# 0xC0000054/pdn-jpegxl

Hardware: AMD Instinct MI355X
Metric: megapixels/sec decode (4K lossy VarDCT) (higher is better)
Workload: dtype f32

## Files before the change

pdn_jpegxl_amd/csrc/decoder.cc:

```cpp
#include <hip/hip_runtime.h>
#include <algorithm>
#include <atomic>
#include <cmath>
#include <cstdarg>
#include <cstdio>
#include <cstdlib>
#include <cstring>
#include <memory>
#include <mutex>
#include <string>
#include <thread>
#include <vector>
#include "../../include/jxlfiletypeio.h"
#include "host_parse.h"
#include "icc.h"
#include "kernels.h"

namespace jxlhip {

struct HipError : std::runtime_error {
  explicit HipError(const std::string& m) : std::runtime_error(m) {}
};
#define HIP_OK(expr)                                                                                      \
  do {                                                                                                    \
// ... 77 lines not shown
  hipStream_t own_stream = nullptr;
  float* d_basis_all = nullptr;
  float* d_basis_small = nullptr;
  float* d_basis_mfma = nullptr;
  float* d_llf_scale = nullptr;
  uint16_t* d_natural[kNumOrders] = {};
  U32x2* d_scan[kNumQuantTables] = {};
  float* d_dq[kNumQuantTables] = {};
  uint32_t dq_n[kNumQuantTables] = {};
  struct Tap { std::vector<uint8_t> qcoef[3], xyb_idct[3], xyb_filtered[3], noise_rnd[3], noise[3]; };
  struct Slot {
    uint8_t* d_ws = nullptr; size_t ws_cap = 0;
    uint8_t* d_blob = nullptr; size_t blob_cap = 0;
    uint8_t* h_blob = nullptr; size_t h_blob_cap = 0;
    uint32_t* h_status = nullptr; size_t h_status_cap = 0;
    int n = 0;
    std::vector<ParsedFrame> frames;
    int nfiles = 0;
    std::vector<int> file_of;
    std::vector<ParsedFrame> files;
    std::vector<DevImage> imgs;
    std::vector<int> parse_status;
    std::vector<std::string> parse_msg;
    std::vector<size_t> status_off;
    DevImage* d_imgs = nullptr;
    bool pending = false;
    hipEvent_t lf_done = nullptr, hf_done = nullptr, done = nullptr, uploaded = nullptr;
    std::vector<Tap> taps;
    std::vector<std::string> stage_names;
    std::vector<int> stage_chain;
    std::vector<hipEvent_t> events;
    std::vector<float> stage_ms;
  };
  static constexpr int kSlots = 3;
  static constexpr int kPixelChunk = 32;
  Slot slots[kSlots];
  int cur = 0, last = 0;
  Slot* active = &slots[0];
  hipStream_t stream_lf = nullptr;
  hipStream_t stream_hf = nullptr;
  hipStream_t last_stream = nullptr;
  std::vector<std::string> total_names;
  std::vector<double> total_ms;
  int total_batches = 0;
  std::string sticky_error;
  int sticky_status = 0;
  uint8_t* li_dev = nullptr; uint8_t* li_host = nullptr; size_t li_cap = 0;
  void EnsureLoadImageBuffers(size_t bytes);
  int lane_stride_override = 0;
  int hf_stride_override = 0;
  bool debug_taps = false;
  int band_first_row = 0, band_rows = 0;
  bool no_stream_pairs = false;
  bool no_direct = false, mod_lanes64 = false;
  bool overlap = true;

  explicit JxlHipDecoder(int dev);
  ~JxlHipDecoder();
  void EnsureWs(size_t bytes);
  void EnsureBlob(size_t bytes);
  void Mark(const char* name, hipStream_t s, int chain);
  void WaitSlot(Slot& S);
  Slot& Last() { return slots[last]; }
  void Decode(int32_t n_, const uint8_t* const* host_data, const size_t* sizes, const uint8_t* const* dev_data,
              uint8_t* const* dev_out, hipStream_t stream, bool sync, DecoderStatus* statuses, ErrorInfo* err);
  DecoderStatus Finish(DecoderStatus* statuses, ErrorInfo* err);
  void CopyPlaneTap(int stage);
  void PrepassSingle(ParsedFrame& f, const uint8_t* dev_file);
};

JxlHipDecoder::JxlHipDecoder(int dev) {
  if (dev < 0) HIP_OK(hipGetDevice(&dev));
  device = dev;
  HIP_OK(hipSetDevice(device));
  int entropy_cus = 0, pixel_cus = 0;
  if (const char* e = Knob("JXLHIP_ENTROPY_CUS")) entropy_cus = std::min(256, std::max(0, atoi(e)));
  if (const char* e = Knob("JXLHIP_PIXEL_CUS")) pixel_cus = std::min(256, std::max(0, atoi(e)));
  auto masked_stream = [](hipStream_t* s, int first, int count) {
    uint32_t mask[8] = {0, 0, 0, 0, 0, 0, 0, 0};
    for (int i = first; i < first + count; i++) mask[i >> 5] |= 1u << (i & 31);
    HIP_OK(hipExtStreamCreateWithCUMask(s, 8, mask));
  };
  if (pixel_cus) masked_stream(&own_stream, 256 - pixel_cus, pixel_cus);
  else HIP_OK(hipStreamCreateWithFlags(&own_stream, hipStreamNonBlocking));
  int prio_least = 0, prio_greatest = 0;
  (void)hipDeviceGetStreamPriorityRange(&prio_least, &prio_greatest);
  const int prio = Knob("JXLHIP_NO_PRIORITY") ? prio_least : prio_greatest;
  if (entropy_cus) {
    masked_stream(&stream_lf, 0, entropy_cus);
    masked_stream(&stream_hf, 0, entropy_cus);
  } else {
    HIP_OK(hipStreamCreateWithPriority(&stream_lf, hipStreamNonBlocking, prio));
    HIP_OK(hipStreamCreateWithPriority(&stream_hf, hipStreamNonBlocking, prio));
  }
  for (auto& S : slots) {
    HIP_OK(hipEventCreateWithFlags(&S.lf_done, hipEventDisableTiming));
    HIP_OK(hipEventCreateWithFlags(&S.hf_done, hipEventDisableTiming));
    HIP_OK(hipEventCreateWithFlags(&S.done, hipEventDisableTiming));
    HIP_OK(hipEventCreateWithFlags(&S.uploaded, hipEventDisableTiming));
  }
  if (const char* e = Knob("JXLHIP_NO_OVERLAP")) overlap = atoi(e) == 0;
  const StaticTables& st = GetStaticTables();
  std::vector<float> all;
  for (int i = 0; i < 6; i++) all.insert(all.end(), st.basis[i].begin(), st.basis[i].end());
  HIP_OK(hipMalloc(&d_basis_all, all.size() * 4));
  HIP_OK(hipMemcpy(d_basis_all, all.data(), all.size() * 4, hipMemcpyHostToDevice));
// ... 1026 lines not shown
      }
    }
  }
  if (!patch_tiles.empty()) {
    PatchFrame* pfr = (PatchFrame*)(h_blob + off_patch_frames);
    for (size_t k = 0; k < patch_image.size(); k++) {
      const ParsedFrame& f = frames[patch_image[k]];
      PatchFrame& p = pfr[k];
      memset(&p, 0, sizeof(p));
      p.px = (float*)imgs[patch_image[k]].out;
      p.w = (int32_t)f.xsize; p.h = (int32_t)f.ysize;
      p.has_alpha = f.alpha_index >= 0 ? 1 : 0;
      p.nch = f.ncolor + p.has_alpha;
      p.premul = (p.has_alpha && f.ec[f.alpha_index].alpha_associated) ? 1 : 0;
    }
    for (size_t k = 0; k < patch_refs.size(); k++) {
      const HostPatchRef& s = patch_src[k];
      const ParsedFrame& a = frames[s.atlas];
      const size_t nch = a.ncolor + (a.alpha_index >= 0 ? 1 : 0);
      patch_refs[k].px = (const float*)imgs[s.atlas].out + ((size_t)s.y0 * a.xsize + s.x0) * nch;
      patch_refs[k].stride = (int32_t)a.xsize;
    }
    memcpy(h_blob + off_patch_refs, patch_refs.data(), sizeof(PatchRef) * patch_refs.size());
    memcpy(h_blob + off_patch_pos, patch_pos.data(), sizeof(PatchPos) * patch_pos.size());
    memcpy(h_blob + off_patch_tiles, patch_tiles.data(), sizeof(PatchTile) * patch_tiles.size());
    memcpy(h_blob + off_patch_list, patch_list.data(), sizeof(int32_t) * patch_list.size());
  }
  memcpy(h_blob + off_imgs, imgs.data(), sizeof(DevImage) * imgs.size());
  d_imgs = (DevImage*)(d_blob + off_imgs);
  stage_names.clear();
  S.stage_chain.clear();
  Mark("start", s_lf, 0);
  static const int skip_stages = Knob("JXLHIP_SKIP_STAGES") ? atoi(Knob("JXLHIP_SKIP_STAGES")) : 0;
  if (!(skip_stages & 1)) HIP_OK(hipMemsetAsync(d_ws, 0, zero_bytes, s_lf));
  HIP_OK(hipMemcpyAsync(d_blob, h_blob, blob.off, hipMemcpyHostToDevice, s_lf));
  Mark("upload+clear", s_lf, 0);
  const bool pix_on_hf = Knob("JXLHIP_PIX_ON_HF") && s_hf != stream;
  const bool early_noise = any_noise && !debug_taps && s_lf != stream && !pix_on_hf;
  if (early_noise) {
    HIP_OK(hipEventRecord(S.uploaded, s_lf));
    HIP_OK(hipStreamWaitEvent(stream, S.uploaded, 0));
    Mark("noise_start", stream, 3);
    LaunchNoise(d_imgs, std::min(pixel_chunk, n), max_groups, max_w, max_h, stream);
    Mark("noise", stream, 3);
  }
  const int direct_lf = global_direct && lf_per_wave == 1, direct_alpha = global_direct && per_alpha_wg == 1;
  bool lean_mod = true;
  for (int i = 0; i < n; i++)
    if (parse_status[i] == DecoderStatus_Ok && frames[i].encoding == 0 &&
        (!frames[i].tree_row_static || frames[i].tree_uses_wp || frames[i].mcode.use_prefix || frames[i].mcode.lz77)) lean_mod = false;
  if (!(skip_stages & 1)) {
  LaunchLfAns(d_imgs, (const SectionTask*)(d_blob + off_lf_ans_tasks), nlf_ans_t, lf_per_wave, lds_lf <= kLdsMax ? lds_lf : 0, direct_lf, lean_mod, s_lf);
  Mark("lf_ans", s_lf, 0);
  LaunchLfFinish(d_imgs, (const SectionTask*)(d_blob + off_lf_tasks), nlf_t, s_lf);
  LaunchHfBlockList(d_imgs, n, max_groups, s_lf);
  LaunchLfPixelStages(d_imgs, n, max_cells, s_lf);
  }
  Mark("lf_finish+pixels", s_lf, 0);
  if (s_lf != s_hf) {
    HIP_OK(hipEventRecord(S.lf_done, s_lf));
    HIP_OK(hipStreamWaitEvent(s_hf, S.lf_done, 0));
  }
#ifdef JXLHIP_EXPERIMENTS
  if (const char* e = Knob("JXLHIP_INTERFERE")) {
    int kind = 0, wgs = 1, lds_kb = 64; float ms = 100.f;
    if (sscanf(e, "%d,%d,%d,%f", &kind, &wgs, &lds_kb, &ms) >= 1 && kind >= 1 && kind <= 6 && wgs >= 1 && wgs <= 16 && lds_kb >= 1 && lds_kb <= 160 && ms > 0 && ms < 2000) {
      static hipStream_t xs = nullptr;
      static float* xbuf = nullptr;
      const size_t xbytes = (size_t)512 << 20;
      if (!xs) { HIP_OK(hipStreamCreateWithFlags(&xs, hipStreamNonBlocking)); HIP_OK(hipMalloc(&xbuf, xbytes)); }
      if (s_lf != s_hf) HIP_OK(hipStreamWaitEvent(xs, S.lf_done, 0));
      LaunchInterference(kind, wgs, lds_kb, ms, xbuf, xbytes, xs);
    }
  }
#endif
  Mark("hf_start", s_hf, 1);
  if (!(skip_stages & 2))
  LaunchHfDecode(d_imgs, (const SectionTask*)(d_blob + off_pass_tasks), npass_t, hf_waves * 64, lane_stride, hf_ring, lds_hf <= kLdsMax ? lds_hf : 0, lds_hf_lanes, s_hf);
  Mark("hf_decode", s_hf, 1);
  if (any_alpha && !(skip_stages & 4))
    LaunchAlphaAns(d_imgs, (const SectionTask*)(d_blob + off_alpha_tasks), nalpha_t, alpha_stride, lds_alpha <= kLdsMax ? lds_alpha : 0, direct_alpha, lean_mod, s_hf);
  Mark("alpha_ans", s_hf, 1);
  if (debug_taps) {
    taps.assign(n, Tap());
    LaunchExpandCoefficients(d_imgs, n, true, max_tiles, stream);
    HIP_OK(hipStreamSynchronize(stream));
    CopyPlaneTap(0);
  }
  const bool finish_on_hf = s_hf == stream || debug_taps || !Knob("JXLHIP_ALPHA_FINISH_ON_PIX");
  if (finish_on_hf) {
    if (any_alpha && !(skip_stages & 4)) LaunchAlphaFinish(d_imgs, n, max_groups, s_hf);
    Mark("alpha_finish", s_hf, 1);
  }
  if (s_hf != stream) {
    HIP_OK(hipEventRecord(S.hf_done, s_hf));
    HIP_OK(hipStreamWaitEvent(stream, S.hf_done, 0));
  }
  Mark("main_start", stream, 2);
  if (!finish_on_hf) {
    if (any_alpha && !(skip_stages & 4)) LaunchAlphaFinish(d_imgs, n, max_groups, stream);
    Mark("alpha_finish", stream, 2);
  }
  hipStream_t s_pix = pix_on_hf ? s_hf : stream;
  for (int c0 = 0; c0 < n; c0 += pixel_chunk) {
    const int cnt = std::min(pixel_chunk, n - c0);
    if (!(skip_stages & 8))
    LaunchReconTiles(d_imgs + c0, cnt, max_tiles, d_basis_all, d_basis_small, d_llf_scale, d_basis_mfma, s_pix);
// ... 257 lines not shown
    info->has_alpha = f.alpha_index >= 0;
    info->num_channels = f.ncolor + (f.black_index >= 0 ? 1 : 0) + info->has_alpha;
    info->bytes_per_sample = (int32_t)OutBytesPerSample(f);
    info->reserved = f.exp_bits ? 1 : 0;
    info->xsize_blocks = f.w8; info->ysize_blocks = f.h8;
    info->num_groups = f.ng; info->num_lf_groups = f.nlf;
    info->epf_iters = f.epf_iters; info->gaborish = f.gab;
    info->codestream_bytes = f.cs_size;
    return DecoderStatus_Ok;
  } catch (const ParseError& e) {
    SetErr(err, "%s", e.what());
    return e.status;
  } catch (const std::exception& e) {
    SetErr(err, "%s", e.what());
    return DecoderStatus_DecodeError;
  }
}

DecoderStatus jxlhip_decode_batch(JxlHipDecoder* dec, int32_t n, const uint8_t* const* host_data, const size_t* sizes,
                                  const uint8_t* const* dev_data, uint8_t* const* dev_out, void* stream, int32_t synchronize,
                                  DecoderStatus* statuses, ErrorInfo* err) {
  if (!dec || !host_data || !sizes || !dev_out || n <= 0) return DecoderStatus_NullParameter;
  try {
    dec->Decode(n, host_data, sizes, dev_data, dev_out, (hipStream_t)stream, synchronize != 0, statuses, err);
    if (statuses) for (int i = 0; i < n; i++) if (statuses[i] != DecoderStatus_Ok) return statuses[i];
    return DecoderStatus_Ok;
  } catch (const std::bad_alloc&) {
    return DecoderStatus_OutOfMemory;
  } catch (const std::exception& e) {
    SetErr(err, "%s", e.what());
    return DecoderStatus_DecodeError;
  }
}

DecoderStatus jxlhip_finish(JxlHipDecoder* dec, DecoderStatus* statuses, ErrorInfo* err) {
  if (!dec) return DecoderStatus_NullParameter;
  try {
    return dec->Finish(statuses, err);
  } catch (const std::exception& e) {
    SetErr(err, "%s", e.what());
    return DecoderStatus_DecodeError;
  }
}

int32_t jxlhip_set_option(JxlHipDecoder* dec, const char* name, int32_t value) {
  if (!dec || !name) return 0;
  if (!strcmp(name, "debug_taps")) { dec->debug_taps = value != 0; return 1; }
  if (!strcmp(name, "query_pixel_chunk")) return JxlHipDecoder::kPixelChunk;
  if (!strcmp(name, "lane_stride")) { if (value != 0 && !PowerOfTwoUpTo64(value)) return 0; dec->lane_stride_override = value; return 1; }
  if (!strcmp(name, "band_first_row")) { if (value < 0) return 0; dec->band_first_row = value; return 1; }
  if (!strcmp(name, "band_rows")) { if (value < 0) return 0; dec->band_rows = value; return 1; }
  if (!strcmp(name, "no_direct")) { dec->no_direct = value != 0; return 1; }
  if (!strcmp(name, "no_stream_pairs")) { dec->no_stream_pairs = value != 0; return 1; }
  if (!strcmp(name, "mod_lanes64")) { dec->mod_lanes64 = value != 0; return 1; }
  if (!strcmp(name, "overlap")) { dec->overlap = value != 0; return 1; }
  return 0;
}

size_t jxlhip_read_plane(JxlHipDecoder* dec, int32_t index, const char* name, int32_t channel, void* dst, size_t capacity) {
  if (!dec || !name) return 0;
  JxlHipDecoder::Slot& S = dec->Last();
  if (index < 0 || index >= S.n || S.pending) return 0;
  if (S.parse_status[index] != DecoderStatus_Ok) return 0;
  const DevImage& d = S.imgs[index];
  std::string nm(name);
  const size_t cells = (size_t)d.w8 * d.h8, pix = (size_t)d.wp * d.hp;
  const void* src = nullptr;
  size_t bytes = 0;
  bool host = false;
  const int c = std::min(2, std::max(0, channel));
  if (nm == "lf") { src = d.lf_final[c]; bytes = cells * 4; }
  else if (nm == "lf_quant") { src = d.lfq[c]; bytes = cells * 4; }
  else if (nm == "cellinfo") { src = d.cellinfo; bytes = cells * 4; }
  else if (nm == "raw_quant") { src = d.rawq; bytes = cells * 2; }
  else if (nm == "sharpness") { src = d.sharp; bytes = cells; }
  else if (nm == "ytox") { src = d.ytox; bytes = (size_t)d.wt * d.ht; }
  else if (nm == "ytob") { src = d.ytob; bytes = (size_t)d.wt * d.ht; }
  else if (nm == "alpha") { src = d.alpha; bytes = (size_t)d.w * d.h; }
  else if (nm == "inv_sigma") { src = d.inv_sigma; bytes = cells * 4; }
  else if (dec->debug_taps && (size_t)index < S.taps.size()) {
    host = true;
    if (nm == "qcoef") { src = S.taps[index].qcoef[c].data(); bytes = S.taps[index].qcoef[c].size(); }
    else if (nm == "xyb_idct") { src = S.taps[index].xyb_idct[c].data(); bytes = S.taps[index].xyb_idct[c].size(); }
    else if (nm == "xyb_filtered") { src = S.taps[index].xyb_filtered[c].data(); bytes = S.taps[index].xyb_filtered[c].size(); }
    else if (nm == "noise_rnd") { src = S.taps[index].noise_rnd[c].data(); bytes = S.taps[index].noise_rnd[c].size(); }
    else if (nm == "noise") { src = S.taps[index].noise[c].data(); bytes = S.taps[index].noise[c].size(); }
  }
  (void)pix;
  if (!src || !bytes) return 0;
  if (dst && capacity) {
    size_t nb = std::min(bytes, capacity);
    if (host) memcpy(dst, src, nb);
    else if (hipMemcpy(dst, src, nb, hipMemcpyDeviceToHost) != hipSuccess) return 0;
  }
  return bytes;
}

int32_t jxlhip_stage_times(JxlHipDecoder* dec, const char** names, float* ms, int32_t capacity) {
  if (!dec) return 0;
  JxlHipDecoder::Slot& S = dec->Last();
  int32_t k = 0;
  for (size_t i = 1; i < S.stage_names.size() && i < S.stage_ms.size() && k < capacity; i++) {
    if (S.stage_ms[i] < 0.f) continue;
    if (names) names[k] = S.stage_names[i].c_str();
    if (ms) ms[k] = S.stage_ms[i];
    k++;
// ... 209 lines not shown
```

pdn_jpegxl_amd/csrc/entropy_kernels.hip:

```cpp
#include <hip/hip_runtime.h>
#include <cstdlib>
#include "dev_types.h"
#include "dev_util.h"
#include "kernels.h"

namespace jxlhip {

namespace {

__device__ const uint8_t d_order_bucket[kNumStrategies] = {0, 1, 1, 1, 2, 3, 4, 4, 5, 5, 6, 6, 1, 1, 1, 1, 1, 1, 7, 8, 8, 9, 10, 10, 11, 12, 12};
__device__ const uint8_t d_log2cx[kNumStrategies] = {0, 0, 0, 0, 1, 2, 0, 1, 0, 2, 1, 2, 0, 0, 0, 0, 0, 0, 3, 2, 3, 4, 3, 4, 5, 4, 5};
__device__ const uint8_t d_log2cy[kNumStrategies] = {0, 0, 0, 0, 1, 2, 1, 0, 2, 0, 2, 1, 0, 0, 0, 0, 0, 0, 3, 3, 2, 4, 4, 3, 5, 5, 4};
__device__ const uint8_t d_nnz_ctx[64] = {0,   0,   31,  62,  62,  93,  93,  93,  93,  123, 123, 123, 123, 152, 152, 152, 152, 152, 152, 152, 152, 180,
                                          180, 180, 180, 180, 180, 180, 180, 180, 180, 180, 180, 206, 206, 206, 206, 206, 206, 206, 206, 206, 206, 206,
                                          206, 206, 206, 206, 206, 206, 206, 206, 206, 206, 206, 206, 206, 206, 206, 206, 206, 206, 206, 206};

__device__ __forceinline__ int CeilLog2D(uint32_t x) { return x <= 1 ? 0 : 32 - __clz(x - 1); }
__device__ __forceinline__ int32_t UnpackSigned(uint32_t u) { return (int32_t)(u >> 1) ^ -(int32_t)(u & 1); }
#ifndef JXLHIP_PRIO_SERIAL
#define JXLHIP_PRIO_SERIAL 0
#endif
#if JXLHIP_PRIO_SERIAL
#define JXL_SERIAL_PRIO() __builtin_amdgcn_s_setprio(JXLHIP_PRIO_SERIAL)
#else
// ... 1013 lines not shown
      if (b.Read(4) != 3) { err |= kErrUnsupportedHeader; break; }
      b.SetLz(lzw, 20, max(max((uint32_t)tw, count), (uint32_t)bw));
      b.lz_copy = 0; b.lz_done = 0;
      state = InitAnsState(b, mt.tab);
    }
    int chan, sid, w, h, stride;
    int32_t* out;
    ChanDesc* cd = desc + max(i, 0);
    if (i < 0) {
      chan = 0; sid = 0; w = im.w; h = im.h; stride = im.w; out = im.alpha32; cd = im.alpha_desc;
    } else if (i < 3) {
      const int c = i == 0 ? 1 : (i == 1 ? 0 : 2);
      chan = i; sid = 1 + g; w = bw; h = bh; stride = im.w8;
      out = im.lfq[c] + (size_t)by0 * im.w8 + bx0;
    } else {
      chan = i - 3; sid = sid_meta;
      if (i < 5) { w = tw; h = th; stride = tw; out = scratch + (i - 3) * 1024; }
      else if (i == 5) { w = (int)count; h = 2; stride = (int)count; out = scratch + 2048; }
      else { w = bw; h = bh; stride = bw; out = scratch + 2048 + 2 * 65536; }
    }
    DecodeChannelLane<kLds, false, kGeneric>(b, state, mt.tab, mt.tree, chan, sid, w, h, out, stride, cd, wps);
  }
  if (!err && (state != 0x130000u || b.slow_err || start_bits + b.Consumed() > (im.sec_off[lf_sec] + im.sec_size[lf_sec]) * 8)) err |= kErrBitstream;
  if (im.single) im.lf_end_bits[0] = start_bits + b.Consumed();
  im.lf_count[g] = err ? 0u : count;
  if (err) SetError(im, err, 1, g);
}

__global__ __launch_bounds__(256) void lf_finish_kernel(const DevImage* __restrict__ imgs, const SectionTask* tasks) {
  __shared__ int32_t s_carry[4][256];
  __shared__ uint32_t s_count, s_flag;
  __shared__ uint32_t s_part[256];
  __shared__ uint32_t s_cov[256 * 8];
  const DevImage& im = imgs[tasks[blockIdx.x].image];
  const int g = tasks[blockIdx.x].first;
  const uint32_t count = im.lf_count[g];
  if (!count) return;
  const int tid = threadIdx.x, wave = tid >> 6, lane = tid & 63;
  const int gx = g % im.xlf, gy = g / im.xlf;
  const int bx0 = gx * kLfGroupBlocks, by0 = gy * kLfGroupBlocks;
  const int bw = min(kLfGroupBlocks, im.w8 - bx0), bh = min(kLfGroupBlocks, im.h8 - by0);
  const int tw = (bw + 7) / 8, th = (bh + 7) / 8;
  int32_t* scratch = im.binfo + (size_t)g * kBinfoInts;
  int32_t* s_x = scratch;
  int32_t* s_b = scratch + 1024;
  int32_t* s_info = scratch + 2048;
  int32_t* s_sharp = scratch + 2048 + 2 * 65536;
  const ChanDesc* desc = im.lf_desc + (size_t)g * 8;
  const I4* tree = (const I4*)im.tree;
  const int sid_meta = 1 + 2 * im.nlf + g;
  JXL_LDS int32_t* carry = (JXL_LDS int32_t*)s_carry[wave];
  if (wave < 3) {
    const int chan_of[3] = {1, 0, 2};
    FinishChannelI32(desc[wave], tree, wave, 1 + g, im.lfq[chan_of[wave]] + (size_t)by0 * im.w8 + bx0, im.w8, bw, bh, carry, lane);
  } else {
    FinishChannelI32(desc[3], tree, 0, sid_meta, s_x, tw, tw, th, carry, lane);
    FinishChannelI32(desc[4], tree, 1, sid_meta, s_b, tw, tw, th, carry, lane);
    FinishChannelI32(desc[5], tree, 2, sid_meta, s_info, (int)count, (int)count, 2, carry, lane);
    FinishChannelI32(desc[6], tree, 3, sid_meta, s_sharp, bw, bw, bh, carry, lane);
  }
  __threadfence_block();
  __syncthreads();
  uint32_t err = 0;
  const int tx0 = bx0 / 8, ty0 = by0 / 8;
  for (int i = tid; i < tw * th; i += 256) {
    const int x = i % tw, y = i / tw;
    const int vx = s_x[i], vb = s_b[i];
    if (vx < -128 || vx > 127 || vb < -128 || vb > 127) err |= kErrRange;
    im.ytox[(size_t)(ty0 + y) * im.wt + tx0 + x] = (int8_t)vx;
    im.ytob[(size_t)(ty0 + y) * im.wt + tx0 + x] = (int8_t)vb;
  }
  for (int i = tid; i < bw * bh; i += 256) {
    const int x = i % bw, y = i / bw;
    int sh = s_sharp[i];
    if (sh < 0 || sh > 7) { err |= kErrRange; sh = 0; }
    im.sharp[(size_t)(by0 + y) * im.w8 + bx0 + x] = (uint8_t)sh;
  }
  __syncthreads();
  int32_t* s_pos = s_sharp;
  uint32_t* const s_pre = (uint32_t*)(scratch + 2048 + 3 * 65536);
  if (tid == 0) { s_count = 0; s_flag = 0; }
  for (int i = tid; i < 256 * 8; i += 256) s_cov[i] = 0;
  {
    const uint32_t per = (count + 255) / 256, i0 = min(count, (uint32_t)tid * per), i1 = min(count, i0 + per);
    uint32_t sum = 0;
    for (uint32_t i = i0; i < i1; i++) {
      const int es = s_info[i], eq = 1 + s_info[count + i];
      const bool ok = es >= 0 && es < kNumStrategies && eq >= 1 && eq <= 256;
      if (!ok) err |= kErrBlockLayout;
      if (es >= 14 && es <= 17) err |= kErrUnsupportedTransform | kErrBlockLayout;
      sum += ok ? 1u << d_log2cx[es] : 1u;
    }
    s_part[tid] = sum;
    __syncthreads();
    if (tid == 0) {
      uint32_t acc = 0;
      for (int i = 0; i < 256; i++) { const uint32_t v = s_part[i]; s_part[i] = acc; acc += v; }
      s_pre[count] = acc;
    }
    __syncthreads();
    uint32_t base = s_part[tid];
    for (uint32_t i = i0; i < i1; i++) {
      const int es = s_info[i];
      s_pre[i] = base;
      base += (es >= 0 && es < kNumStrategies) ? 1u << d_log2cx[es] : 1u;
    }
    if (err & kErrBlockLayout) atomicOr(&s_flag, 1u);
// ... 658 lines not shown
      }
      typedef uint32_t __attribute__((ext_vector_type(4))) U4v;
      *(JXL_GLB U4v*)(out + (size_t)r * im.w + q * 16) = U4v{pk[0], pk[1], pk[2], pk[3]};
    }
  }
}

__global__ __launch_bounds__(64, 3) void alpha_finish_kernel(const DevImage* __restrict__ imgs) {
  __shared__ int32_t s_carry[256];
  __shared__ int32_t s_tile[64 * 65];
  const DevImage& im = imgs[blockIdx.y];
  const int g = blockIdx.x;
  if (!im.has_alpha || g >= im.ng || im.is_modular) return;
  const int lane = threadIdx.x;
  const int gx = g % im.xg, gy = g / im.xg;
  if (gy * kGroupDim >= im.band_y1 || (gy + 1) * kGroupDim <= im.band_y0) return;
  const ChanDesc d = im.alpha_desc[g];
  const int x0 = gx * kGroupDim, y0 = gy * kGroupDim;
  const int gw = min(kGroupDim, im.w - x0), gh = min(kGroupDim, im.h - y0);
  int32_t* plane = im.alpha32 + (size_t)y0 * im.w + x0;
  const int sid = im.alpha_in_global ? 0 : 1 + 3 * im.nlf + kNumQuantTables + g;
  if (d.pad0 == 1) return;
  if (im.out_bits == 8 && im.alpha_bits == 8 && !im.alpha_exp) {
    uint8_t* out = im.alpha + (size_t)y0 * im.w + x0;
    if (d.kind == kChanResid) {
      PredictWaveTiled<true>((const I4*)im.tree, 0, sid, plane, im.w, gw, gh, d.kind, d.value, out, im.w, (JXL_LDS int32_t*)s_carry,
                             (JXL_LDS int32_t*)s_tile, lane);
    } else {
      const bool cst = d.kind == kChanConst;
      const uint8_t cv = (uint8_t)(d.value < 0 ? 0 : (d.value > 255 ? 255 : d.value));
      for (int y = 0; y < gh; y++) {
        const size_t ro = (size_t)y * im.w;
        for (int x = lane; x < gw; x += 64) {
          const int v = cst ? 0 : plane[ro + x];
          out[ro + x] = cst ? cv : (uint8_t)(v < 0 ? 0 : (v > 255 ? 255 : v));
        }
      }
    }
    return;
  }
  if (d.kind == kChanResid)
    PredictWaveTiled<false>((const I4*)im.tree, 0, sid, plane, im.w, gw, gh, d.kind, d.value, nullptr, 0, (JXL_LDS int32_t*)s_carry,
                            (JXL_LDS int32_t*)s_tile, lane);
  __builtin_amdgcn_fence(__ATOMIC_ACQ_REL, "workgroup");
  __syncthreads();
  const bool cst = d.kind == kChanConst;
  for (int i = lane; i < gw * gh; i += 64) {
    const size_t o = (size_t)(i / gw) * im.w + (i % gw);
    const uint32_t v = SampleToOutBits(cst ? d.value : plane[o], im.alpha_bits, im.alpha_exp, im.out_bits, im.out_float);
    StoreOutSample(im.alpha, (size_t)y0 * im.w + x0 + o, v, im.out_bits);
  }
}

struct ModRect { int x0, y0, w, h; };
__device__ __forceinline__ bool ModSectionRect(const DevImage& im, int kind, int g, const ModChanDev& ch, int c, ModRect* r) {
  if (kind == 0) {
    if (c >= im.mod_first_group) return false;
    r->x0 = 0; r->y0 = 0; r->w = ch.w; r->h = ch.h;
    return ch.w > 0 && ch.h > 0;
  }
  if (c < im.mod_first_group) return false;
  const int shift = min(ch.hshift, ch.vshift);
  if (kind == 1 ? shift < 3 : shift > 2) return false;
  const int dim = kind == 1 ? im.group_dim * 8 : im.group_dim;
  const int gx = kind == 1 ? g % im.xlf : g % im.xg, gy = kind == 1 ? g / im.xlf : g / im.xg;
  const int x0 = (gx * dim) >> ch.hshift, y0 = (gy * dim) >> ch.vshift;
  const int w = max(0, min(dim >> ch.hshift, ch.w - x0)), h = max(0, min(dim >> ch.vshift, ch.h - y0));
  r->x0 = x0; r->y0 = y0; r->w = w; r->h = h;
  return w > 0 && h > 0;
}
__device__ __forceinline__ void ModSectionOf(const DevImage& im, int s, int* kind, int* g, int* sid, int* sec) {
  if (s == 0) { *kind = 0; *g = 0; *sid = 0; *sec = 0; }
  else if (s <= im.nlf) { *kind = 1; *g = s - 1; *sid = 1 + im.nlf + *g; *sec = 1 + *g; }
  else { *kind = 2; *g = s - 1 - im.nlf; *sid = 1 + 3 * im.nlf + kNumQuantTables + *g; *sec = 2 + im.nlf + *g; }
}

template <bool kLds, bool kUni = false>
__global__ __launch_bounds__(64) void modular_ans_kernel(const DevImage* imgs, const SectionTask* tasks, int lanes, int rb_width, int wp_lds, int scalar_rows) {
  JXL_SERIAL_PRIO();
  extern __shared__ __align__(16) uint8_t smem[];
  const SectionTask task = tasks[blockIdx.x];
  const DevImage& im = imgs[task.image];
  const size_t off_rows = (size_t)64 * kRingWords * 4;
  const size_t off_wp = off_rows + (size_t)(kUni ? 3 : lanes) * rb_width * 4;
  const size_t wp_ints = (size_t)10 * (rb_width + 2);
  const size_t off_grid = off_wp + (wp_lds ? (size_t)lanes * wp_ints * 4 : 0);
  const size_t off_tab = off_grid + (kUni ? (size_t)kUniGridCells * 16 : 0);
  ModTables<kLds> mt;
  LoadModTables<kLds>(im, smem, off_tab, mt, threadIdx.x, 64, lanes == 1 && scalar_rows);
  const int lane = kUni ? 0 : (int)threadIdx.x;
  if (lane >= task.count || lane >= lanes) return;
  RowBuf<kLds> rows;
  rows.rb = (typename AS<kLds>::Row)((JXL_LDS int32_t*)((JXL_LDS uint8_t*)smem + off_rows) + lane);
  rows.rb_stride = lanes;
  rows.rb_width = rb_width;
  int32_t* const wp_local = wp_lds ? (int32_t*)(smem + off_wp) + (size_t)lane * wp_ints : nullptr;
  UniAreas uni;
  if constexpr (kUni) {
    uni.rows = (JXL_LDS int32_t*)((JXL_LDS uint8_t*)smem + off_rows);
    uni.wp = wp_lds ? (JXL_LDS int32_t*)((JXL_LDS uint8_t*)smem + off_wp) : nullptr;
    uni.grid = (JXL_LDS uint32_t*)((JXL_LDS uint8_t*)smem + off_grid);
    uni.rw = rb_width;
    uni.use_wp = im.wp_grp != nullptr && wp_lds;
  }
  const int s0 = task.first + lane;
  const int nsub = im.single ? 3 : 1;
// ... 150 lines not shown
        a = R; b = G; c = B;
      } else {
        if (custom & 1) c += a;
        if ((custom >> 1) == 1) b += a;
        else if ((custom >> 1) == 2) b += (a + c) >> 1;
      }
      int32_t o[3];
      o[perm % 3] = a;
      o[(perm + 1 + perm / 3) % 3] = b;
      o[(perm + 2 - perm / 3) % 3] = c;
      v[bc] = o[0]; v[bc + 1] = o[1]; v[bc + 2] = o[2];
    }
    const int ncol = im.ncolor;
    float unmul = 1.0f;
    if (im.unpremultiply) {
      int32_t av = 0;
      for (int c = ncol; c < nch; c++) if (im.mod_out_pos[c] == nch - 1) av = v[c];
      const float af = im.alpha_exp ? BitsToFloatSample(av, im.alpha_bits) : (float)av * im.alpha_unit;
      unmul = 1.0f / fmaxf(1.0f / 67108864.0f, af);
    }
    for (int c = 0; c < nch; c++) {
      const int pos = im.mod_out_pos[c];
      const bool is_alpha = im.has_alpha && pos == nch - 1;
      const bool is_black = im.cmyk && pos == 3;
      uint32_t s = SampleToOutBits(v[c], c < ncol ? im.sample_bits : (is_alpha ? im.alpha_bits : im.black_bits), c < ncol ? im.sample_exp : (is_alpha ? im.alpha_exp : 0),
                                   im.out_bits, im.out_float);
      if (im.unpremultiply && c < ncol) {
        const float f = im.sample_exp ? BitsToFloatSample(v[c], im.sample_bits) : (float)v[c] * (1.0f / (float)((1u << im.sample_bits) - 1));
        s = FloatToOutBits(f * unmul, im.out_bits, im.out_float);
      }
      if (im.cmyk && !is_alpha) { (void)is_black; s = 255u - s; }
      StoreOutSample(im.out, i * nch + pos, s, im.out_bits);
    }
  }
}

static void RaiseLds(const void* fn, size_t bytes) {
  if (bytes > 48 * 1024) (void)hipFuncSetAttribute(fn, hipFuncAttributeMaxDynamicSharedMemorySize, (int)bytes);
}

void LaunchLfAns(const DevImage* imgs, const SectionTask* tasks, int ntasks, int slots, size_t lds_bytes, int scalar_rows, bool lean, hipStream_t s) {
  if (ntasks <= 0) return;
  if (lds_bytes && lean) {
    RaiseLds((const void*)lf_ans_kernel<true, false>, lds_bytes);
    hipLaunchKernelGGL((lf_ans_kernel<true, false>), dim3(ntasks), dim3(64), lds_bytes, s, imgs, tasks, slots, scalar_rows);
  } else if (lds_bytes) {
    RaiseLds((const void*)lf_ans_kernel<true>, lds_bytes);
    hipLaunchKernelGGL(lf_ans_kernel<true>, dim3(ntasks), dim3(64), lds_bytes, s, imgs, tasks, slots, scalar_rows);
  } else {
    hipLaunchKernelGGL(lf_ans_kernel<false>, dim3(ntasks), dim3(64), (size_t)slots * kRingWords * 4, s, imgs, tasks, slots, 0);
  }
}

void LaunchLfFinish(const DevImage* imgs, const SectionTask* tasks, int ntasks, hipStream_t s) {
  if (ntasks <= 0) return;
  hipLaunchKernelGGL(lf_finish_kernel, dim3(ntasks), dim3(256), 0, s, imgs, tasks);
}

void LaunchHfBlockList(const DevImage* imgs, int nimg, int max_groups, hipStream_t s) {
  if (nimg <= 0 || max_groups <= 0) return;
  hipLaunchKernelGGL(hf_blocklist_kernel, dim3(max_groups, nimg), dim3(64), 0, s, imgs);
}

size_t HfLaneLdsBytes(int ring_words) { return 96 + (size_t)ring_words * 4 + (size_t)(ring_words / 2) * 4; }

void LaunchHfDecode(const DevImage* imgs, const SectionTask* tasks, int nwg, int threads, int lane_stride, int ring_words,
                    size_t lds_bytes, size_t lane_bytes, hipStream_t s) {
  if (nwg <= 0) return;
  (void)ring_words;
  if (lds_bytes) {
    RaiseLds((const void*)hf_decode_kernel<true, 32>, lds_bytes);
    hipLaunchKernelGGL((hf_decode_kernel<true, 32>), dim3(nwg), dim3(threads), lds_bytes, s, imgs, tasks, lane_stride);
  } else {
    RaiseLds((const void*)hf_decode_kernel<false, 32>, lane_bytes);
    hipLaunchKernelGGL((hf_decode_kernel<false, 32>), dim3(nwg), dim3(threads), lane_bytes, s, imgs, tasks, lane_stride);
  }
}

void LaunchAlphaAns(const DevImage* imgs, const SectionTask* tasks, int nwg, int lane_stride, size_t lds_bytes, int scalar_rows, bool lean, hipStream_t s) {
  if (nwg <= 0) return;
  if (lds_bytes && lean) {
    RaiseLds((const void*)alpha_ans_kernel<true, false>, lds_bytes);
    hipLaunchKernelGGL((alpha_ans_kernel<true, false>), dim3(nwg), dim3(64), lds_bytes, s, imgs, tasks, lane_stride, scalar_rows);
  } else if (lds_bytes) {
    RaiseLds((const void*)alpha_ans_kernel<true>, lds_bytes);
    hipLaunchKernelGGL(alpha_ans_kernel<true>, dim3(nwg), dim3(64), lds_bytes, s, imgs, tasks, lane_stride, scalar_rows);
  } else {
    hipLaunchKernelGGL(alpha_ans_kernel<false>, dim3(nwg), dim3(64), (size_t)(64 / lane_stride) * kRingWords * 4, s, imgs, tasks, lane_stride, 0);
  }
}

void LaunchModularAns(const DevImage* imgs, int nimg, const SectionTask* tasks, int ntasks, size_t lds_bytes, int max_sections, int max_coded,
                      int lanes, int rb_width, int wp_lds, int scalar_rows, hipStream_t s) {
  if (ntasks <= 0) return;
  if (lds_bytes && lanes == 1 && rb_width > 0) {
    RaiseLds((const void*)modular_ans_kernel<true, true>, lds_bytes);
    hipLaunchKernelGGL((modular_ans_kernel<true, true>), dim3(ntasks), dim3(64), lds_bytes, s, imgs, tasks, lanes, rb_width, wp_lds, scalar_rows);
  } else if (lds_bytes) {
    RaiseLds((const void*)modular_ans_kernel<true>, lds_bytes);
    hipLaunchKernelGGL(modular_ans_kernel<true>, dim3(ntasks), dim3(64), lds_bytes, s, imgs, tasks, lanes, rb_width, wp_lds, scalar_rows);
  } else {
    const size_t lds = (size_t)64 * kRingWords * 4 + (size_t)lanes * rb_width * 4 + (wp_lds ? (size_t)lanes * 10 * (rb_width + 2) * 4 : 0);
    RaiseLds((const void*)modular_ans_kernel<false>, lds);
    hipLaunchKernelGGL(modular_ans_kernel<false>, dim3(ntasks), dim3(64), lds, s, imgs, tasks, lanes, rb_width, wp_lds, 0);
  }
  hipLaunchKernelGGL(modular_finish_kernel, dim3(max_sections * max_coded, nimg), dim3(64), 0, s, imgs, max_coded);
}

// ... 49 lines not shown
```

pdn_jpegxl_amd/csrc/kernels.h:

```cpp
#pragma once
#include <hip/hip_runtime.h>
#include "dev_types.h"

namespace jxlhip {

void LaunchLfAns(const DevImage* imgs, const SectionTask* tasks, int ntasks, int slots, size_t lds_bytes, int scalar_rows, bool lean, hipStream_t s);
void LaunchLfFinish(const DevImage* imgs, const SectionTask* tasks, int ntasks, hipStream_t s);
void LaunchHfBlockList(const DevImage* imgs, int nimg, int max_groups, hipStream_t s);
size_t HfLaneLdsBytes(int ring_words);
void LaunchHfDecode(const DevImage* imgs, const SectionTask* tasks, int nwg, int threads, int lane_stride, int ring_words, size_t lds_bytes,
                    size_t lane_bytes, hipStream_t s);
void LaunchAlphaAns(const DevImage* imgs, const SectionTask* tasks, int nwg, int lane_stride, size_t lds_bytes, int scalar_rows, bool lean, hipStream_t s);
void LaunchAlphaFinish(const DevImage* imgs, int nimg, int max_groups, hipStream_t s);
void LaunchModularAns(const DevImage* imgs, int nimg, const SectionTask* tasks, int ntasks, size_t lds_bytes, int max_sections, int max_coded,
                      int lanes, int rb_width, int wp_lds, int scalar_rows, hipStream_t s);
void LaunchModularOp(int kind, int32_t* a, int32_t* b, int32_t* c, int aw, int ah, int rw, int rh, int type, hipStream_t s);
void LaunchModularPalette(const int32_t* palette, const int32_t* index, int32_t* const* out, int nout, int nb_colors, int w, int h, uint32_t* status,
                          hipStream_t s);
void LaunchModularOut(const DevImage* imgs, int nimg, size_t max_pixels, hipStream_t s);
void LaunchOrient(const uint8_t* src, uint8_t* dst, int w, int h, int px_bytes, int orientation, hipStream_t s);
void LaunchLfPixelStages(const DevImage* imgs, int nimg, size_t max_cells, hipStream_t s);
void LaunchExpandCoefficients(const DevImage* imgs, int nimg, bool all_tiles, int max_tiles, hipStream_t s);
void LaunchGenericReconstruct(const DevImage* imgs, int nimg, const float* basis_all, const float* basis_small,
                              const float* llf_scale, hipStream_t s);
void LaunchReconTiles(const DevImage* imgs, int nimg, int max_tiles, const float* basis_all, const float* basis_small,
                      const float* llf_scale, const float* basis_mfma, hipStream_t s);
void LaunchFilterTiles(const DevImage* imgs, int nimg, int max_w, int max_h, int stage_mask, bool any_unfiltered,
                       int any_fused, int any_fused2, hipStream_t s);

void LaunchNoise(const DevImage* imgs, int nimg, int max_groups, int max_w, int max_h, hipStream_t s);

void LaunchCompose(const ComposeImage* imgs, const ComposeFrame* frames, int nimg, int max_segments, hipStream_t s);
void LaunchPatches(const PatchFrame* frames, const PatchTile* tiles, int ntiles, const int32_t* list, const PatchPos* pos, const PatchRef* refs,
                   hipStream_t s);

void LaunchStatusToHost(const uint32_t* src, uint32_t* dst_pinned, int nwords, hipStream_t s);
#ifdef JXLHIP_EXPERIMENTS
void LaunchInterference(int kind, int wg_per_cu, int lds_kb, float ms, float* scratch, size_t scratch_bytes, hipStream_t s);
#endif

}
```

Baseline: 30310.

## Add wavefront-pipelined LF gradient finish kernel for pure-gradient channels

Adds a dedicated kernel that reconstructs LF quantized channels whose modular tree always selects the clamped-gradient predictor. It uses a diagonal wavefront over 16-wide row segments, passing north neighbours between lanes and using vectorized loads and stores where alignment allows. Channels it handles are marked so the generic lf_finish_kernel skips them. The intent is to replace the slow serial per-row finish with a pipelined parallel one. In exchange it adds an extra launch and a per-row tree check, and correctness depends on the cross-lane neighbour logic.

After: 31770 (median of 6 runs). +4.8%, better.

```diff
diff --git a/pdn_jpegxl_amd/csrc/decoder.cc b/pdn_jpegxl_amd/csrc/decoder.cc
--- a/pdn_jpegxl_amd/csrc/decoder.cc
+++ b/pdn_jpegxl_amd/csrc/decoder.cc
@@ -153,6 +153,7 @@
   bool debug_taps = false;
   int band_first_row = 0, band_rows = 0;
   bool no_stream_pairs = false;
+  bool no_lf_pipeline = false;
   bool no_direct = false, mod_lanes64 = false;
   bool overlap = true;
 
@@ -1285,7 +1286,7 @@
   if (!(skip_stages & 1)) {
   LaunchLfAns(d_imgs, (const SectionTask*)(d_blob + off_lf_ans_tasks), nlf_ans_t, lf_per_wave, lds_lf <= kLdsMax ? lds_lf : 0, direct_lf, lean_mod, s_lf);
   Mark("lf_ans", s_lf, 0);
-  LaunchLfFinish(d_imgs, (const SectionTask*)(d_blob + off_lf_tasks), nlf_t, s_lf);
+  LaunchLfFinish(d_imgs, (const SectionTask*)(d_blob + off_lf_tasks), nlf_t, !no_lf_pipeline, s_lf);
   LaunchHfBlockList(d_imgs, n, max_groups, s_lf);
   LaunchLfPixelStages(d_imgs, n, max_cells, s_lf);
   }
@@ -1649,6 +1650,7 @@
   if (!strcmp(name, "band_rows")) { if (value < 0) return 0; dec->band_rows = value; return 1; }
   if (!strcmp(name, "no_direct")) { dec->no_direct = value != 0; return 1; }
   if (!strcmp(name, "no_stream_pairs")) { dec->no_stream_pairs = value != 0; return 1; }
+  if (!strcmp(name, "no_lf_pipeline")) { dec->no_lf_pipeline = value != 0; return 1; }
   if (!strcmp(name, "mod_lanes64")) { dec->mod_lanes64 = value != 0; return 1; }
   if (!strcmp(name, "overlap")) { dec->overlap = value != 0; return 1; }
   return 0;
diff --git a/pdn_jpegxl_amd/csrc/entropy_kernels.hip b/pdn_jpegxl_amd/csrc/entropy_kernels.hip
--- a/pdn_jpegxl_amd/csrc/entropy_kernels.hip
+++ b/pdn_jpegxl_amd/csrc/entropy_kernels.hip
@@ -1089,7 +1089,8 @@
   JXL_LDS int32_t* carry = (JXL_LDS int32_t*)s_carry[wave];
   if (wave < 3) {
     const int chan_of[3] = {1, 0, 2};
-    FinishChannelI32(desc[wave], tree, wave, 1 + g, im.lfq[chan_of[wave]] + (size_t)by0 * im.w8 + bx0, im.w8, bw, bh, carry, lane);
+    if (desc[wave].pad0 != 1)
+      FinishChannelI32(desc[wave], tree, wave, 1 + g, im.lfq[chan_of[wave]] + (size_t)by0 * im.w8 + bx0, im.w8, bw, bh, carry, lane);
   } else {
     FinishChannelI32(desc[3], tree, 0, sid_meta, s_x, tw, tw, th, carry, lane);
     FinishChannelI32(desc[4], tree, 1, sid_meta, s_b, tw, tw, th, carry, lane);
@@ -1854,6 +1855,114 @@
   }
 }
 
+template <bool kVec>
+__device__ __forceinline__ void LfGradientSteps(JXL_GLB int32_t* const plane, const int stride, const int bw, const int rows, const int nq,
+                                                const int steps, const int li) {
+  typedef int32_t __attribute__((ext_vector_type(4))) I4v;
+  auto line_of = [&](int T, int* r_out, int* q_out) {
+    const int m = T - li;
+    const int r = (m >> 4) * 16 + li, q = m & 15;
+    *r_out = r; *q_out = q;
+    return m >= 0 && r < rows && q < nq;
+  };
+  auto load_line = [&](int T, I4v* v) {
+    int r, q;
+    const bool act = line_of(T, &r, &q);
+    const JXL_GLB int32_t* const row = plane + (size_t)(act ? r : 0) * stride;
+    const int x = act ? q * 16 : 0;
+    if constexpr (kVec) {
+#pragma unroll
+      for (int k = 0; k < 4; k++) v[k] = *(const JXL_GLB I4v*)(row + min(x + 4 * k, bw - 4));
+    } else {
+#pragma unroll
+      for (int j = 0; j < 16; j++) v[j >> 2][j & 3] = row[min(x + j, bw - 1)];
+    }
+  };
+  I4v cur[4], nxt[4];
+  load_line(0, nxt);
+  int32_t prev_out[16];
+#pragma unroll
+  for (int j = 0; j < 16; j++) prev_out[j] = 0;
+  int32_t W = 0, n_last = 0;
+  for (int T = 0; T < steps; T++) {
+#pragma unroll
+    for (int k = 0; k < 4; k++) cur[k] = nxt[k];
+    load_line(T + 1, nxt);
+    int r, q;
+    const bool act = line_of(T, &r, &q);
+    int32_t nq16[16];
+#pragma unroll
+    for (int j = 0; j < 16; j++) nq16[j] = RowRotateFromBelow(prev_out[j]);
+    const bool top = r == 0;
+    int32_t o[16];
+#pragma unroll
+    for (int j = 0; j < 16; j++) {
+      const int32_t res = cur[j >> 2][j & 3];
+      int32_t n, nw;
+      if (top) { n = W; nw = W; }
+      else { n = nq16[j]; nw = j == 0 ? n_last : nq16[j - 1]; }
+      if (j == 0 && q == 0) {
+        const int32_t w0 = top ? 0 : nq16[0];
+        W = w0; n = w0; nw = w0;
+      }
+      const int32_t val = (int32_t)((uint32_t)res + (uint32_t)ClampedGradient32(W, n, nw));
+      o[j] = val;
+      W = val;
+    }
+    n_last = nq16[15];
+    if (act) {
+#pragma unroll
+      for (int j = 0; j < 16; j++) prev_out[j] = o[j];
+      JXL_GLB int32_t* const dst = plane + (size_t)r * stride + q * 16;
+      const int left = bw - q * 16;
+      if constexpr (kVec) {
+#pragma unroll
+        for (int k = 0; k < 4; k++)
+          if (4 * k < left) *(JXL_GLB I4v*)(dst + 4 * k) = I4v{o[4 * k], o[4 * k + 1], o[4 * k + 2], o[4 * k + 3]};
+      } else {
+#pragma unroll
+        for (int j = 0; j < 16; j++)
+          if (j < left) dst[j] = o[j];
+      }
+    }
+  }
+}
+
+__global__ __launch_bounds__(64) void lf_finish_gradient_kernel(const DevImage* __restrict__ imgs, const SectionTask* tasks) {
+  const DevImage& im = imgs[tasks[blockIdx.x].image];
+  const int g = tasks[blockIdx.x].first;
+  if (!im.lf_count[g]) return;
+  const int lane = threadIdx.x, sub = lane >> 4, li = lane & 15;
+  const int gx = g % im.xlf, gy = g / im.xlf;
+  const int bx0 = gx * kLfGroupBlocks, by0 = gy * kLfGroupBlocks;
+  const int bw = min(kLfGroupBlocks, im.w8 - bx0), bh = min(kLfGroupBlocks, im.h8 - by0);
+  if (bw <= 0 || bh <= 0) return;
+  const int chan = min(sub, 2);
+  const int c = chan == 0 ? 1 : (chan == 1 ? 0 : 2);
+  bool mine = sub < 3 && im.lf_desc[(size_t)g * 8 + chan].kind == kChanResid;
+  if (mine) {
+    const I4* tree = (const I4*)im.tree;
+    for (int r = li; r < bh; r += 16) {
+      bool used_y = false;
+      mine = mine && (RowNode(tree, chan, 1 + g, r, &used_y).a & 0xFF) == 5;
+      if (!used_y) break;
+    }
+  }
+  {
+    const uint64_t bal = __ballot(mine);
+    mine = ((bal >> (sub * 16)) & 0xFFFFu) == 0xFFFFu;
+  }
+  if (__ballot(mine) == 0) return;
+  JXL_GLB int32_t* const plane = G(im.lfq[c]) + (size_t)by0 * im.w8 + bx0;
+  const int rows = mine ? bh : 0, nq = mine ? (bw + 15) >> 4 : 0;
+  int steps = mine ? rows + nq - 1 : 0;
+  steps = max(steps, __shfl_xor(steps, 16)); steps = max(steps, __shfl_xor(steps, 32));
+  if (mine && li == 0) im.lf_desc[(size_t)g * 8 + chan].pad0 = 1;
+  const bool vec = (im.w8 & 3) == 0 && (((uintptr_t)im.lfq[0] | (uintptr_t)im.lfq[1] | (uintptr_t)im.lfq[2]) & 15) == 0;
+  if (vec) LfGradientSteps<true>(plane, im.w8, bw, rows, nq, steps, li);
+  else LfGradientSteps<false>(plane, im.w8, bw, rows, nq, steps, li);
+}
+
 struct ModRect { int x0, y0, w, h; };
 __device__ __forceinline__ bool ModSectionRect(const DevImage& im, int kind, int g, const ModChanDev& ch, int c, ModRect* r) {
   if (kind == 0) {
@@ -2110,8 +2219,9 @@
   }
 }
 
-void LaunchLfFinish(const DevImage* imgs, const SectionTask* tasks, int ntasks, hipStream_t s) {
+void LaunchLfFinish(const DevImage* imgs, const SectionTask* tasks, int ntasks, bool pipeline, hipStream_t s) {
   if (ntasks <= 0) return;
+  if (pipeline) hipLaunchKernelGGL(lf_finish_gradient_kernel, dim3(ntasks), dim3(64), 0, s, imgs, tasks);
   hipLaunchKernelGGL(lf_finish_kernel, dim3(ntasks), dim3(256), 0, s, imgs, tasks);
 }
 
diff --git a/pdn_jpegxl_amd/csrc/kernels.h b/pdn_jpegxl_amd/csrc/kernels.h
--- a/pdn_jpegxl_amd/csrc/kernels.h
+++ b/pdn_jpegxl_amd/csrc/kernels.h
@@ -5,7 +5,7 @@
 namespace jxlhip {
 
 void LaunchLfAns(const DevImage* imgs, const SectionTask* tasks, int ntasks, int slots, size_t lds_bytes, int scalar_rows, bool lean, hipStream_t s);
-void LaunchLfFinish(const DevImage* imgs, const SectionTask* tasks, int ntasks, hipStream_t s);
+void LaunchLfFinish(const DevImage* imgs, const SectionTask* tasks, int ntasks, bool pipeline, hipStream_t s);
 void LaunchHfBlockList(const DevImage* imgs, int nimg, int max_groups, hipStream_t s);
 size_t HfLaneLdsBytes(int ring_words);
 void LaunchHfDecode(const DevImage* imgs, const SectionTask* tasks, int nwg, int threads, int lane_stride, int ring_words, size_t lds_bytes,
```
